# InternetMaximalism/plonky2_bn254

Measured on NVIDIA B200. Metric: g1_scalar_mul_stark_proofs_per_sec, higher is better.
Workload: dtype u64

## Files before the change

### plonky2_bn254_b200/csrc/merkle.cuh

```cuda
#pragma once
#include "poseidon.cuh"
#include "poseidon_tc.cuh"

namespace merkle {

using poseidon::Digest;

struct LeafHashK {
  const u64* lde;
  size_t stride;
  int W, log_n;
  Digest* out;
  int natural = 0;
  PB_HD void operator()(size_t j) const {
    u64 s[12];
#pragma unroll
    for (int i = 0; i < 12; i++) s[i] = 0;
    if (W <= 4) {
      for (int c = 0; c < W; c++) s[c] = lde[(size_t)c * stride + j];
    } else {
      int c = 0;
      for (; c + 8 <= W; c += 8) {
#pragma unroll
        for (int k = 0; k < 8; k++) s[k] = lde[(size_t)(c + k) * stride + j];
        poseidon::permute(s);
      }
      if (c < W) {
        for (int k = 0; c + k < W; k++) s[k] = lde[(size_t)(c + k) * stride + j];
        poseidon::permute(s);
      }
    }
    Digest d;
#pragma unroll
    for (int i = 0; i < 4; i++) d.e[i] = s[i];
    out[natural ? j : (size_t)gl::brev32((u32)j, log_n)] = d;
  }
};

struct RowHashK {
  const u64* rows;
  int len;
  Digest* out;
  PB_HD void operator()(size_t i) const {
    u64 s[12];
#pragma unroll
    for (int k = 0; k < 12; k++) s[k] = 0;
    const u64* row = rows + i * (size_t)len;
    if (len <= 4) {
      for (int c = 0; c < len; c++) s[c] = row[c];
    } else {
      for (int c = 0; c < len; c += 8) {
        for (int k = 0; k < 8 && c + k < len; k++) s[k] = row[c + k];
        poseidon::permute(s);
      }
    }
    Digest d;
#pragma unroll
    for (int k = 0; k < 4; k++) d.e[k] = s[k];
    out[i] = d;
  }
};

struct LevelK {
  const Digest* child;
  Digest* parent;
  PB_HD void operator()(size_t i) const { parent[i] = poseidon::two_to_one(child[2 * i], child[2 * i + 1]); }
};

#if !PB_HOSTSIM
__device__ __forceinline__ void stage_rc2(u64* rc2) {
  for (int i = threadIdx.x; i < poseidon::RC2_WORDS; i += blockDim.x) rc2[i] = poseidon::RC2_DEV[i];
  __syncthreads();
}

__global__ void __launch_bounds__(poseidon::tc::CTA, poseidon::tc::CTAS_PER_SM)
    k_leaf_hash_tc(const u64* __restrict__ lde, size_t stride, int W, int log_n, Digest* __restrict__ out, size_t rows,
                   int natural) {
  extern __shared__ unsigned char tc_dyn[];
  __shared__ u64 tc_bar;
  __shared__ u32 tc_slot[2];
  poseidon::tc::Ctx ctx;
  poseidon::tc::setup(ctx, tc_dyn, &tc_bar, tc_slot);
  const size_t j = (size_t)blockIdx.x * blockDim.x + threadIdx.x;
  const bool live = j < rows;
  const u64* p = lde + (live ? j : 0);
  u64 s[12];
#pragma unroll
  for (int i = 0; i < 12; i++) s[i] = 0;
  const int chunks = (W + 7) / 8;
#pragma unroll 1
  for (int c = 0; c < chunks; c++) {
    const int len = W - 8 * c;
    const u64* q = p + (size_t)c * 8 * stride;
#pragma unroll
    for (int k = 0; k < 8; k++)
      if (k < len) s[k] = q[(size_t)k * stride];
    poseidon::tc::permute(s, ctx);
  }
  if (live) {
    Digest d;
#pragma unroll
    for (int i = 0; i < 4; i++) d.e[i] = s[i];
    out[natural ? j : (size_t)gl::brev32((u32)j, log_n)] = d;
  }
  poseidon::tc::teardown(ctx);
}

__global__ void __launch_bounds__(128, 6) k_level(const Digest* __restrict__ child, Digest* __restrict__ parent, size_t n) {
  __shared__ __align__(16) u64 rc2[poseidon::RC2_WORDS];
  stage_rc2(rc2);
  const size_t i = (size_t)blockIdx.x * blockDim.x + threadIdx.x;
  if (i >= n) return;
  u64 s[12];
  const Digest l = child[2 * i], r = child[2 * i + 1];
#pragma unroll
  for (int k = 0; k < 4; k++) {
    s[k] = l.e[k];
    s[4 + k] = r.e[k];
    s[8 + k] = 0;
  }
  poseidon::lazy::permute(s, rc2);
  Digest d;
#pragma unroll
  for (int k = 0; k < 4; k++) d.e[k] = s[k];
  parent[i] = d;
}
#endif

static inline size_t tree_digests(int log_n, int cap_height) {
  size_t total = 0;
  for (int l = log_n; l >= cap_height; l--) total += (size_t)1 << l;
  return total;
}
static inline size_t level_offset(int log_n, int lvl) {
  size_t off = 0;
  for (int l = 0; l < lvl; l++) off += (size_t)1 << (log_n - l);
  return off;
}

static inline void launch_level(const Digest* child, Digest* parent, size_t n, pbStream s) {
#if PB_HOSTSIM
  LevelK k{child, parent};
  pb_launch("merkle level", k, n, s, 128);
#else
  k_level<<<(unsigned)((n + 127) / 128), 128, 0, s>>>(child, parent, n);
  g_pb_launches++;
  pb_check_last("merkle level");
#endif
}
static inline void build_levels(Digest* digests, int log_n, int cap_height, pbStream s) {
  if (cap_height > log_n) throw Pb254Error(6, "merkle: cap_height > log2(leaves)");
  size_t off = 0;
  for (int l = 0; l < log_n - cap_height; l++) {
    size_t m = (size_t)1 << (log_n - l);
    launch_level(digests + off, digests + off + m, m / 2, s);
    off += m;
  }
}

static inline void build_from_lde(const u64* lde, size_t stride, int W, int log_n, int cap_height, Digest* digests,
                                  pbStream s) {
#if PB_HOSTSIM
  LeafHashK k{lde, stride, W, log_n, digests};
  pb_launch("leaf hash", k, (size_t)1 << log_n, s, 128);
#else
  if (W <= 4) {
    LeafHashK k{lde, stride, W, log_n, digests};
    pb_launch("leaf copy", k, (size_t)1 << log_n, s, 128);
  } else {
    const size_t n = (size_t)1 << log_n;
    k_leaf_hash_tc<<<(unsigned)((n + 127) / 128), poseidon::tc::CTA, poseidon::tc::SMEM_BYTES, s>>>(lde, stride, W, log_n,
                                                                                                  digests, n, 0);
    g_pb_launches++;
    pb_check_last("leaf hash");
  }
#endif
  build_levels(digests, log_n, cap_height, s);
}
static inline void build_from_rows(const u64* rows, int len, int log_n, int cap_height, Digest* digests, pbStream s) {
  RowHashK k{rows, len, digests};
  pb_launch("row hash", k, (size_t)1 << log_n, s, 128);
  build_levels(digests, log_n, cap_height, s);
}


static inline void hash_rows_natural(const u64* m, size_t stride, int W, size_t rows, Digest* out, pbStream s) {
#if PB_HOSTSIM
  LeafHashK k{m, stride, W, 0, out, 1};
  pb_launch("leaf hash (rows)", k, rows, s, 128);
#else
  if (W <= 4) {
    LeafHashK k{m, stride, W, 0, out, 1};
    pb_launch("leaf copy (rows)", k, rows, s, 128);
  } else {
    k_leaf_hash_tc<<<(unsigned)((rows + 127) / 128), poseidon::tc::CTA, poseidon::tc::SMEM_BYTES, s>>>(m, stride, W, 0, out,
                                                                                                     rows, 1);
    g_pb_launches++;
    pb_check_last("leaf hash (rows)");
  }
#endif
}
struct SubtreeLeavesK {
  const Digest* all;
  Digest* leaves;
  size_t first;
  int log_N;
  PB_HD void operator()(size_t q) const { leaves[q] = all[gl::brev32((u32)(first + q), log_N)]; }
};

}
```

### plonky2_bn254_b200/csrc/poseidon_tc.cuh

```cuda
#pragma once
#include "poseidon.cuh"

#if !PB_HOSTSIM
namespace poseidon {
namespace tc {

static constexpr int CTA = 128;
static constexpr int A_BYTES = 128 * 128;
static constexpr int B_BYTES = 96 * 128;
static constexpr int CTAS_PER_SM = 5;
static constexpr int SMEM_BYTES = 41 * 1024;
static_assert(A_BYTES + 2 * B_BYTES + 1024 <= SMEM_BYTES && SMEM_BYTES <= 48 * 1024, "shared-memory plan");
__host__ __device__ constexpr u32 idesc(u32 n) { return (2u << 4) | ((n >> 3) << 17) | ((128u >> 4) << 24); }

static __device__ const uint4 B_IMAGE[B_BYTES / 16] = {
#include "poseidon_constants_tcb.inc"
};
static __device__ const uint4 BF_IMAGE[B_BYTES / 16] = {
#include "poseidon_constants_tcf.inc"
};

__device__ __forceinline__ u32 smem_u32(const void* p) { return (u32)__cvta_generic_to_shared(p); }

__device__ __forceinline__ u64 smem_desc(u32 addr) {
  return (u64)((addr & 0x3FFFFu) >> 4) | ((u64)(1024u >> 4) << 32) | (1ull << 46) | (2ull << 61);
}

struct Ctx {
  unsigned char* row;
  u32 r7;
  u32 bar;
  u32 tmem0, tmem1;
  u64 adesc, bdesc, bfdesc;
  u32 parity;
};

__device__ __forceinline__ void setup(Ctx& c, unsigned char* dyn, u64* bar, u32* slot) {
  const u32 t = threadIdx.x;
  unsigned char* base = dyn + ((1024u - (smem_u32(dyn) & 1023u)) & 1023u);
  unsigned char* a = base;
  unsigned char* b = base + A_BYTES;
  unsigned char* bf = b + B_BYTES;
  for (int i = t; i < B_BYTES / 16; i += CTA) {
    reinterpret_cast<uint4*>(b)[i] = B_IMAGE[i];
    reinterpret_cast<uint4*>(bf)[i] = BF_IMAGE[i];
  }
  c.row = a + t * 128;
  c.r7 = t & 7;
  c.bar = smem_u32(bar);
  if (t == 0) {
    asm volatile("mbarrier.init.shared::cta.b64 [%0], 1;" ::"r"(c.bar));
    asm volatile("fence.mbarrier_init.release.cluster;" ::: "memory");
  }
  if (t < 32) {
    asm volatile("tcgen05.alloc.cta_group::1.sync.aligned.shared::cta.b32 [%0], 64;" ::"r"(smem_u32(slot)) : "memory");
    asm volatile("tcgen05.alloc.cta_group::1.sync.aligned.shared::cta.b32 [%0], 32;" ::"r"(smem_u32(slot + 1)) : "memory");
    asm volatile("tcgen05.relinquish_alloc_permit.cta_group::1.sync.aligned;" ::: "memory");
  }
  asm volatile("tcgen05.fence::before_thread_sync;" ::: "memory");
  __syncthreads();
  asm volatile("tcgen05.fence::after_thread_sync;" ::: "memory");
  c.tmem0 = reinterpret_cast<volatile u32*>(slot)[0];
  c.tmem1 = reinterpret_cast<volatile u32*>(slot)[1];
  c.adesc = smem_desc(smem_u32(a));
  c.bdesc = smem_desc(smem_u32(b));
  c.bfdesc = smem_desc(smem_u32(bf));
  c.parity = 0;
}

__device__ __forceinline__ void teardown(const Ctx& c) {
  asm volatile("tcgen05.fence::before_thread_sync;" ::: "memory");
  __syncthreads();
  if (threadIdx.x < 32) {
    asm volatile("tcgen05.dealloc.cta_group::1.sync.aligned.b32 %0, 64;" ::"r"(c.tmem0) : "memory");
    asm volatile("tcgen05.dealloc.cta_group::1.sync.aligned.b32 %0, 32;" ::"r"(c.tmem1) : "memory");
  }
}

template <u32 N>
__device__ __forceinline__ void mma_i8(u32 d_tmem, u64 adesc, u64 bdesc, u32 accumulate) {
  asm volatile(
      "{\n\t"
      ".reg .pred p;\n\t"
      "setp.ne.b32 p, %4, 0;\n\t"
      "tcgen05.mma.cta_group::1.kind::i8 [%0], %1, %2, %3, p;\n\t"
      "}" ::"r"(d_tmem),
      "l"(adesc), "l"(bdesc), "n"(idesc(N)), "r"(accumulate)
      : "memory");
}

#define PB_TMEM_LD32(v, addr)                                                                                       \
  asm volatile(                                                                                                     \
      "tcgen05.ld.sync.aligned.32x32b.x32.b32 {%0, %1, %2, %3, %4, %5, %6, %7, %8, %9, %10, %11, %12, %13, %14, "   \
      "%15, %16, %17, %18, %19, %20, %21, %22, %23, %24, %25, %26, %27, %28, %29, %30, %31}, [%32];"                \
      : "=r"(v[0]), "=r"(v[1]), "=r"(v[2]), "=r"(v[3]), "=r"(v[4]), "=r"(v[5]), "=r"(v[6]), "=r"(v[7]), "=r"(v[8]), \
        "=r"(v[9]), "=r"(v[10]), "=r"(v[11]), "=r"(v[12]), "=r"(v[13]), "=r"(v[14]), "=r"(v[15]), "=r"(v[16]),      \
        "=r"(v[17]), "=r"(v[18]), "=r"(v[19]), "=r"(v[20]), "=r"(v[21]), "=r"(v[22]), "=r"(v[23]), "=r"(v[24]),     \
        "=r"(v[25]), "=r"(v[26]), "=r"(v[27]), "=r"(v[28]), "=r"(v[29]), "=r"(v[30]), "=r"(v[31])                   \
      : "r"(addr)                                                                                                   \
      : "memory")

__device__ __forceinline__ u64 recombine4(u32 acc0, u32 acc1, u32 acc2, u32 acc3) {
  const u32 t1 = __byte_perm(acc1, 0, 0x1044), u1 = __byte_perm(acc1, 0, 0x4432);
  const u32 t3 = __byte_perm(acc3, 0, 0x1044), u3 = __byte_perm(acc3, 0, 0x4432);
  u32 lo, hi;
  asm("{\n\t"
      ".reg .u32 w2, c;\n\t"
      "add.cc.u32   %0, %2, %3;\n\t"
      "addc.u32     %1, %4, %5;\n\t"
      "add.cc.u32   %1, %1, %6;\n\t"
      "addc.u32     w2, %7, 0;\n\t"
      "add.cc.u32   %1, %1, w2;\n\t"
      "addc.u32     c, 0, 0;\n\t"
      "sub.cc.u32   %0, %0, w2;\n\t"
      "subc.u32     %1, %1, 0;\n\t"
      "sub.u32      c, 0, c;\n\t"
      "add.cc.u32   %0, %0, c;\n\t"
      "addc.u32     %1, %1, 0;\n\t"
      "}"
      : "=&r"(lo), "=&r"(hi)
      : "r"(acc0), "r"(t1), "r"(u1), "r"(acc2), "r"(t3), "r"(u3));
  return ((u64)hi << 32) | lo;
}

__device__ __forceinline__ u64 fold8(const u32* q) {
  return recombine4(q[0] + (q[1] << 8), q[2] + (q[3] << 8), q[4] + (q[5] << 8), q[6] + (q[7] << 8));
}


__device__ __forceinline__ u32 onehot(int p, int w) { return (p >> 2) == w ? 1u << ((p & 3) * 8) : 0u; }

__device__ __forceinline__ u32 complement4(const u64 s[12], int i0, int i1, int i2, int i3) {
  const u32 a = __byte_perm((u32)(s[i0] >> 32), (u32)(s[i1] >> 32), 0x0073);
  const u32 b = __byte_perm((u32)(s[i2] >> 32), (u32)(s[i3] >> 32), 0x0073);
  return ~__byte_perm(a, b, 0x5410);
}

__device__ __forceinline__ void product(u64 s[12], Ctx& c, u64 bdesc, uint4 x6, uint4 x7) {
#pragma unroll
  for (int ch = 0; ch < 6; ch++)
    *reinterpret_cast<uint4*>(c.row + ((ch ^ c.r7) << 4)) =
        make_uint4((u32)s[2 * ch], (u32)(s[2 * ch] >> 32), (u32)s[2 * ch + 1], (u32)(s[2 * ch + 1] >> 32));
  *reinterpret_cast<uint4*>(c.row + ((6 ^ c.r7) << 4)) = x6;
  *reinterpret_cast<uint4*>(c.row + ((7 ^ c.r7) << 4)) = x7;
  asm volatile("fence.proxy.async.shared::cta;" ::: "memory");
  asm volatile("tcgen05.fence::before_thread_sync;" ::: "memory");
  __syncthreads();
  if (threadIdx.x == 0) {
    asm volatile("tcgen05.fence::after_thread_sync;" ::: "memory");
#pragma unroll
    for (int k = 0; k < 4; k++) {
      mma_i8<64>(c.tmem0, c.adesc + 2 * k, bdesc + 2 * k, k > 0);
      mma_i8<32>(c.tmem1, c.adesc + 2 * k, bdesc + (64 * 128 >> 4) + 2 * k, k > 0);
    }
    asm volatile("tcgen05.commit.cta_group::1.mbarrier::arrive::one.shared::cluster.b64 [%0];" ::"r"(c.bar) : "memory");
  }
  {
    u32 ok;
    do {
      asm volatile(
          "{\n\t"
          ".reg .pred p;\n\t"
          "mbarrier.try_wait.parity.shared::cta.b64 p, [%1], %2;\n\t"
          "selp.u32 %0, 1, 0, p;\n\t"
          "}"
          : "=r"(ok)
          : "r"(c.bar), "r"(c.parity)
          : "memory");
    } while (!ok);
    c.parity ^= 1;
  }
  asm volatile("tcgen05.fence::after_thread_sync;" ::: "memory");
  {
    const u32 lane_off = ((threadIdx.x >> 5) * 32u) << 16;
    const u32 t0 = c.tmem0 + lane_off, t1 = c.tmem0 + lane_off + 32, t2 = c.tmem1 + lane_off;
#define PB_TC_FOLD(a, base)                                                                                   \
  _Pragma("unroll") for (int r = 0; r < 4; r++) {                                                             \
    const u32* q = a + 8 * r;                                                                                 \
    s[base + r] = fold8(q);                                                                                   \
  }
    u32 a[32], b[32];
    PB_TMEM_LD32(a, t0);
    asm volatile("tcgen05.wait::ld.sync.aligned;" ::: "memory");
    PB_TMEM_LD32(b, t1);
    PB_TC_FOLD(a, 0)
    asm volatile("tcgen05.wait::ld.sync.aligned;" ::: "memory");
    PB_TMEM_LD32(a, t2);
    PB_TC_FOLD(b, 4)
    asm volatile("tcgen05.wait::ld.sync.aligned;" ::: "memory");
    PB_TC_FOLD(a, 8)
#undef PB_TC_FOLD
  }
}

__device__ __forceinline__ void permute(u64 s[12], Ctx& c) {
#pragma unroll
  for (int i = 0; i < 12; i++) {
    const u64 k = RC_DEV[i];
    u64 t = s[i] + k;
    if (t < k) t += gl::EPS;
    s[i] = t;
  }
  constexpr int N_FUSED = N_PARTIAL / 2, N_LAYERS = 2 * HALF_FULL + N_FUSED;
#pragma unroll 1
  for (int L = 0; L < N_LAYERS; L++) {
    uint4 x6, x7;
    u64 bdesc;
    if (L < HALF_FULL || L >= HALF_FULL + N_FUSED) {
#pragma unroll 1
      for (int j = 0; j < 2; j++) {
        u64 t[6];
#pragma unroll
        for (int i = 0; i < 6; i++) t[i] = lazy::sbox(s[i]);
#pragma unroll
        for (int i = 0; i < 6; i++) {
          s[i] = s[i + 6];
          s[i + 6] = t[i];
        }
      }
      const int R = L < HALF_FULL ? L : L + N_FUSED;
      const int p = R < N_ROUNDS - 1 ? R : -1;
      x6 = make_uint4(onehot(p, 0), onehot(p, 1), onehot(p, 2), onehot(p, 3));
      x7 = make_uint4(onehot(p, 4), onehot(p, 5), onehot(p, 6), onehot(p, 7));
      bdesc = c.bdesc;
    } else {
      const int j = L - HALF_FULL, r = HALF_FULL + 2 * j;
      s[0] = lazy::sbox(s[0]);
      u32 X[6][4];
#pragma unroll
      for (int k = 0; k < 6; k++) {
        const u32 a0 = (u32)s[2 * k], a1 = (u32)(s[2 * k] >> 32), b0 = (u32)s[2 * k + 1], b1 = (u32)(s[2 * k + 1] >> 32);
        X[k][0] = __byte_perm(a0, b0, 0x5410);
        X[k][1] = __byte_perm(a0, b0, 0x7632);
        X[k][2] = __byte_perm(a1, b1, 0x5410);
        X[k][3] = __byte_perm(a1, b1, 0x7632);
      }
      const uint4 k0 = *reinterpret_cast<const uint4*>(RC2_DEV + (r + 1) * 24);
      u32 acc[4] = {k0.x, k0.y, k0.z, k0.w};
      lazy::dp_row<0, 0>(acc, X);
      const u64 t = lazy::sbox(recombine4(acc[0], acc[1], acc[2], acc[3]));
      const int p = 8 + j;
      x6 = make_uint4((u32)t, (u32)(t >> 32), onehot(p, 2), onehot(p, 3));
      x7 = make_uint4(onehot(p, 4) | (~(u32)(s[0] >> 32) & 0xFF000000u), complement4(s, 1, 2, 3, 4),
                      complement4(s, 5, 6, 7, 8), complement4(s, 9, 10, 11, 11) & 0x00FFFFFFu);
      bdesc = c.bfdesc;
    }
    product(s, c, bdesc, x6, x7);
  }
#pragma unroll
  for (int i = 0; i < 12; i++) s[i] = s[i] >= gl::P ? s[i] - gl::P : s[i];
}

}
}
#endif
```

Measured before the change: 5.165.

## Interleave two leaf-hash sponges per thread to overlap tensor-core MMA with sbox work

The leaf-hash kernel now processes two rows per thread and ping-pongs their Poseidon permutations. While the tensor-core product for one state is in flight, the threads compute the sboxes for the other, hiding MMA latency and barrier stalls. The grid is halved and register pressure roughly doubles per thread, which may limit occupancy at the unchanged CTAs-per-SM bound.

```diff
diff --git a/plonky2_bn254_b200/csrc/merkle.cuh b/plonky2_bn254_b200/csrc/merkle.cuh
--- a/plonky2_bn254_b200/csrc/merkle.cuh
+++ b/plonky2_bn254_b200/csrc/merkle.cuh
@@ -3,6 +3,9 @@
 #include "poseidon_tc.cuh"
 
 namespace merkle {
+#ifndef LEAF_CTAS_PER_SM
+#define LEAF_CTAS_PER_SM 5
+#endif
 
 using poseidon::Digest;
 
@@ -73,7 +76,8 @@
   __syncthreads();
 }
 
-__global__ void __launch_bounds__(poseidon::tc::CTA, poseidon::tc::CTAS_PER_SM)
+static constexpr unsigned LEAF_ROWS_PER_CTA = 2 * poseidon::tc::CTA;
+__global__ void __launch_bounds__(poseidon::tc::CTA, LEAF_CTAS_PER_SM)
     k_leaf_hash_tc(const u64* __restrict__ lde, size_t stride, int W, int log_n, Digest* __restrict__ out, size_t rows,
                    int natural) {
   extern __shared__ unsigned char tc_dyn[];
@@ -81,27 +85,28 @@
   __shared__ u32 tc_slot[2];
   poseidon::tc::Ctx ctx;
   poseidon::tc::setup(ctx, tc_dyn, &tc_bar, tc_slot);
-  const size_t j = (size_t)blockIdx.x * blockDim.x + threadIdx.x;
-  const bool live = j < rows;
-  const u64* p = lde + (live ? j : 0);
-  u64 s[12];
-#pragma unroll
-  for (int i = 0; i < 12; i++) s[i] = 0;
-  const int chunks = (W + 7) / 8;
-#pragma unroll 1
-  for (int c = 0; c < chunks; c++) {
+  const size_t j0 = (size_t)blockIdx.x * LEAF_ROWS_PER_CTA + threadIdx.x, j1 = j0 + poseidon::tc::CTA;
+  const u64* p0 = lde + (j0 < rows ? j0 : 0);
+  const u64* p1 = lde + (j1 < rows ? j1 : 0);
+  u64 s[2][12];
+#pragma unroll
+  for (int i = 0; i < 12; i++) s[0][i] = s[1][i] = 0;
+  poseidon::tc::sponge2(s, ctx, (W + 7) / 8, [&](int g, int c, u64* sg) {
     const int len = W - 8 * c;
-    const u64* q = p + (size_t)c * 8 * stride;
+    const u64* q = (g ? p1 : p0) + (size_t)c * 8 * stride;
 #pragma unroll
     for (int k = 0; k < 8; k++)
-      if (k < len) s[k] = q[(size_t)k * stride];
-    poseidon::tc::permute(s, ctx);
-  }
-  if (live) {
-    Digest d;
-#pragma unroll
-    for (int i = 0; i < 4; i++) d.e[i] = s[i];
-    out[natural ? j : (size_t)gl::brev32((u32)j, log_n)] = d;
+      if (k < len) sg[k] = q[(size_t)k * stride];
+  });
+#pragma unroll
+  for (int g = 0; g < 2; g++) {
+    const size_t j = g ? j1 : j0;
+    if (j < rows) {
+      Digest d;
+#pragma unroll
+      for (int i = 0; i < 4; i++) d.e[i] = s[g][i];
+      out[natural ? j : (size_t)gl::brev32((u32)j, log_n)] = d;
+    }
   }
   poseidon::tc::teardown(ctx);
 }
@@ -169,7 +174,7 @@
     pb_launch("leaf copy", k, (size_t)1 << log_n, s, 128);
   } else {
     const size_t n = (size_t)1 << log_n;
-    k_leaf_hash_tc<<<(unsigned)((n + 127) / 128), poseidon::tc::CTA, poseidon::tc::SMEM_BYTES, s>>>(lde, stride, W, log_n,
+    k_leaf_hash_tc<<<(unsigned)((n + LEAF_ROWS_PER_CTA - 1) / LEAF_ROWS_PER_CTA), poseidon::tc::CTA, poseidon::tc::SMEM_BYTES, s>>>(lde, stride, W, log_n,
                                                                                                   digests, n, 0);
     g_pb_launches++;
     pb_check_last("leaf hash");
@@ -193,7 +198,7 @@
     LeafHashK k{m, stride, W, 0, out, 1};
     pb_launch("leaf copy (rows)", k, rows, s, 128);
   } else {
-    k_leaf_hash_tc<<<(unsigned)((rows + 127) / 128), poseidon::tc::CTA, poseidon::tc::SMEM_BYTES, s>>>(m, stride, W, 0, out,
+    k_leaf_hash_tc<<<(unsigned)((rows + LEAF_ROWS_PER_CTA - 1) / LEAF_ROWS_PER_CTA), poseidon::tc::CTA, poseidon::tc::SMEM_BYTES, s>>>(m, stride, W, 0, out,
                                                                                                      rows, 1);
     g_pb_launches++;
     pb_check_last("leaf hash (rows)");
diff --git a/plonky2_bn254_b200/csrc/poseidon_tc.cuh b/plonky2_bn254_b200/csrc/poseidon_tc.cuh
--- a/plonky2_bn254_b200/csrc/poseidon_tc.cuh
+++ b/plonky2_bn254_b200/csrc/poseidon_tc.cuh
@@ -136,7 +136,7 @@
   return ~__byte_perm(a, b, 0x5410);
 }
 
-__device__ __forceinline__ void product(u64 s[12], Ctx& c, u64 bdesc, uint4 x6, uint4 x7) {
+__device__ __forceinline__ void store_row(const Ctx& c, const u64 s[12], uint4 x6, uint4 x7) {
 #pragma unroll
   for (int ch = 0; ch < 6; ch++)
     *reinterpret_cast<uint4*>(c.row + ((ch ^ c.r7) << 4)) =
@@ -144,17 +144,19 @@
   *reinterpret_cast<uint4*>(c.row + ((6 ^ c.r7) << 4)) = x6;
   *reinterpret_cast<uint4*>(c.row + ((7 ^ c.r7) << 4)) = x7;
   asm volatile("fence.proxy.async.shared::cta;" ::: "memory");
-  asm volatile("tcgen05.fence::before_thread_sync;" ::: "memory");
-  __syncthreads();
-  if (threadIdx.x == 0) {
-    asm volatile("tcgen05.fence::after_thread_sync;" ::: "memory");
-#pragma unroll
-    for (int k = 0; k < 4; k++) {
-      mma_i8<64>(c.tmem0, c.adesc + 2 * k, bdesc + 2 * k, k > 0);
-      mma_i8<32>(c.tmem1, c.adesc + 2 * k, bdesc + (64 * 128 >> 4) + 2 * k, k > 0);
-    }
-    asm volatile("tcgen05.commit.cta_group::1.mbarrier::arrive::one.shared::cluster.b64 [%0];" ::"r"(c.bar) : "memory");
-  }
+}
+
+__device__ __forceinline__ void issue(const Ctx& c, u64 bdesc) {
+  asm volatile("tcgen05.fence::after_thread_sync;" ::: "memory");
+#pragma unroll
+  for (int k = 0; k < 4; k++) {
+    mma_i8<64>(c.tmem0, c.adesc + 2 * k, bdesc + 2 * k, k > 0);
+    mma_i8<32>(c.tmem1, c.adesc + 2 * k, bdesc + (64 * 128 >> 4) + 2 * k, k > 0);
+  }
+  asm volatile("tcgen05.commit.cta_group::1.mbarrier::arrive::one.shared::cluster.b64 [%0];" ::"r"(c.bar) : "memory");
+}
+
+__device__ __forceinline__ void wait_fold(u64 s[12], Ctx& c) {
   {
     u32 ok;
     do {
@@ -193,7 +195,18 @@
   }
 }
 
-__device__ __forceinline__ void permute(u64 s[12], Ctx& c) {
+__device__ __forceinline__ void product(u64 s[12], Ctx& c, u64 bdesc, uint4 x6, uint4 x7) {
+  store_row(c, s, x6, x7);
+  asm volatile("tcgen05.fence::before_thread_sync;" ::: "memory");
+  __syncthreads();
+  if (threadIdx.x == 0) issue(c, bdesc);
+  wait_fold(s, c);
+}
+
+static constexpr int N_FUSED = N_PARTIAL / 2, N_LAYERS = 2 * HALF_FULL + N_FUSED;
+__host__ __device__ constexpr bool fused_layer(int L) { return L >= HALF_FULL && L < HALF_FULL + N_FUSED; }
+
+__device__ __forceinline__ void add_rc0(u64 s[12]) {
 #pragma unroll
   for (int i = 0; i < 12; i++) {
     const u64 k = RC_DEV[i];
@@ -201,54 +214,127 @@
     if (t < k) t += gl::EPS;
     s[i] = t;
   }
-  constexpr int N_FUSED = N_PARTIAL / 2, N_LAYERS = 2 * HALF_FULL + N_FUSED;
+}
+
+__device__ __forceinline__ void canonicalize(u64 s[12]) {
+#pragma unroll
+  for (int i = 0; i < 12; i++) s[i] = s[i] >= gl::P ? s[i] - gl::P : s[i];
+}
+
+__device__ __forceinline__ u64 layer_sboxes(u64 s[12], int L) {
+  if (!fused_layer(L)) {
+#pragma unroll 1
+    for (int j = 0; j < 2; j++) {
+      u64 t[6];
+#pragma unroll
+      for (int i = 0; i < 6; i++) t[i] = lazy::sbox(s[i]);
+#pragma unroll
+      for (int i = 0; i < 6; i++) {
+        s[i] = s[i + 6];
+        s[i + 6] = t[i];
+      }
+    }
+    return 0;
+  } else {
+    const int j = L - HALF_FULL, r = HALF_FULL + 2 * j;
+    s[0] = lazy::sbox(s[0]);
+    u32 X[6][4];
+#pragma unroll
+    for (int k = 0; k < 6; k++) {
+      const u32 a0 = (u32)s[2 * k], a1 = (u32)(s[2 * k] >> 32), b0 = (u32)s[2 * k + 1], b1 = (u32)(s[2 * k + 1] >> 32);
+      X[k][0] = __byte_perm(a0, b0, 0x5410);
+      X[k][1] = __byte_perm(a0, b0, 0x7632);
+      X[k][2] = __byte_perm(a1, b1, 0x5410);
+      X[k][3] = __byte_perm(a1, b1, 0x7632);
+    }
+    const uint4 k0 = *reinterpret_cast<const uint4*>(RC2_DEV + (r + 1) * 24);
+    u32 acc[4] = {k0.x, k0.y, k0.z, k0.w};
+    lazy::dp_row<0, 0>(acc, X);
+    return lazy::sbox(recombine4(acc[0], acc[1], acc[2], acc[3]));
+  }
+}
+
+__device__ __forceinline__ void layer_tail(const u64 s[12], int L, u64 t, uint4& x6, uint4& x7) {
+  if (!fused_layer(L)) {
+    const int R = L < HALF_FULL ? L : L + N_FUSED;
+    const int p = R < N_ROUNDS - 1 ? R : -1;
+    x6 = make_uint4(onehot(p, 0), onehot(p, 1), onehot(p, 2), onehot(p, 3));
+    x7 = make_uint4(onehot(p, 4), onehot(p, 5), onehot(p, 6), onehot(p, 7));
+  } else {
+    const int p = 8 + L - HALF_FULL;
+    x6 = make_uint4((u32)t, (u32)(t >> 32), onehot(p, 2), onehot(p, 3));
+    x7 = make_uint4(onehot(p, 4) | (~(u32)(s[0] >> 32) & 0xFF000000u), complement4(s, 1, 2, 3, 4),
+                    complement4(s, 5, 6, 7, 8), complement4(s, 9, 10, 11, 11) & 0x00FFFFFFu);
+  }
+}
+
+__device__ __forceinline__ void store_layer(const Ctx& c, const u64 s[12], int L, u64 t) {
+  uint4 x6, x7;
+  layer_tail(s, L, t, x6, x7);
+  store_row(c, s, x6, x7);
+}
+
+__device__ __forceinline__ void permute(u64 s[12], Ctx& c) {
+  add_rc0(s);
 #pragma unroll 1
   for (int L = 0; L < N_LAYERS; L++) {
     uint4 x6, x7;
-    u64 bdesc;
-    if (L < HALF_FULL || L >= HALF_FULL + N_FUSED) {
+    layer_tail(s, L, layer_sboxes(s, L), x6, x7);
+    product(s, c, fused_layer(L) ? c.bfdesc : c.bdesc, x6, x7);
+  }
+  canonicalize(s);
+}
+
+template <class Absorb>
+__device__ __forceinline__ void sponge2(u64 (&s)[2][12], Ctx& c, int chunks, Absorb&& absorb) {
+  u64 t[2];
+#pragma unroll
+  for (int g = 0; g < 2; g++) {
+    absorb(g, 0, s[g]);
+    add_rc0(s[g]);
+    t[g] = layer_sboxes(s[g], 0);
+  }
+  store_layer(c, s[0], 0, t[0]);
+  asm volatile("tcgen05.fence::before_thread_sync;" ::: "memory");
+  __syncthreads();
+  if (threadIdx.x == 0) issue(c, c.bdesc);
+  const int steps = 2 * chunks * N_LAYERS;
+  int L = 0, k = 0;
 #pragma unroll 1
-      for (int j = 0; j < 2; j++) {
-        u64 t[6];
-#pragma unroll
-        for (int i = 0; i < 6; i++) t[i] = lazy::sbox(s[i]);
-#pragma unroll
-        for (int i = 0; i < 6; i++) {
-          s[i] = s[i + 6];
-          s[i + 6] = t[i];
-        }
+  for (int i = 0; i < steps; i++) {
+    const int g = i & 1;
+    const int nL = L + 1 == N_LAYERS ? 0 : L + 1;
+    const bool more = i + 2 < steps;
+    wait_fold(s[0], c);
+    const bool next = i + 1 < steps;
+    if (next) store_layer(c, s[1], g == 0 ? L : nL, t[1]);
+    asm volatile("tcgen05.fence::before_thread_sync;" ::: "memory");
+    __syncthreads();
+    if (threadIdx.x == 0 && next) issue(c, fused_layer(g == 0 ? L : nL) ? c.bfdesc : c.bdesc);
+    if (more) {
+      if (nL == 0) {
+        canonicalize(s[0]);
+        absorb(g, k + 1, s[0]);
+        add_rc0(s[0]);
       }
-      const int R = L < HALF_FULL ? L : L + N_FUSED;
-      const int p = R < N_ROUNDS - 1 ? R : -1;
-      x6 = make_uint4(onehot(p, 0), onehot(p, 1), onehot(p, 2), onehot(p, 3));
-      x7 = make_uint4(onehot(p, 4), onehot(p, 5), onehot(p, 6), onehot(p, 7));
-      bdesc = c.bdesc;
-    } else {
-      const int j = L - HALF_FULL, r = HALF_FULL + 2 * j;
-      s[0] = lazy::sbox(s[0]);
-      u32 X[6][4];
-#pragma unroll
-      for (int k = 0; k < 6; k++) {
-        const u32 a0 = (u32)s[2 * k], a1 = (u32)(s[2 * k] >> 32), b0 = (u32)s[2 * k + 1], b1 = (u32)(s[2 * k + 1] >> 32);
-        X[k][0] = __byte_perm(a0, b0, 0x5410);
-        X[k][1] = __byte_perm(a0, b0, 0x7632);
-        X[k][2] = __byte_perm(a1, b1, 0x5410);
-        X[k][3] = __byte_perm(a1, b1, 0x7632);
-      }
-      const uint4 k0 = *reinterpret_cast<const uint4*>(RC2_DEV + (r + 1) * 24);
-      u32 acc[4] = {k0.x, k0.y, k0.z, k0.w};
-      lazy::dp_row<0, 0>(acc, X);
-      const u64 t = lazy::sbox(recombine4(acc[0], acc[1], acc[2], acc[3]));
-      const int p = 8 + j;
-      x6 = make_uint4((u32)t, (u32)(t >> 32), onehot(p, 2), onehot(p, 3));
-      x7 = make_uint4(onehot(p, 4) | (~(u32)(s[0] >> 32) & 0xFF000000u), complement4(s, 1, 2, 3, 4),
-                      complement4(s, 5, 6, 7, 8), complement4(s, 9, 10, 11, 11) & 0x00FFFFFFu);
-      bdesc = c.bfdesc;
-    }
-    product(s, c, bdesc, x6, x7);
-  }
-#pragma unroll
-  for (int i = 0; i < 12; i++) s[i] = s[i] >= gl::P ? s[i] - gl::P : s[i];
+      t[0] = layer_sboxes(s[0], nL);
+    }
+    if (g == 1) {
+      if (nL == 0) k++;
+      L = nL;
+    }
+#pragma unroll
+    for (int j = 0; j < 12; j++) {
+      const u64 x = s[0][j];
+      s[0][j] = s[1][j];
+      s[1][j] = x;
+    }
+    const u64 x = t[0];
+    t[0] = t[1];
+    t[1] = x;
+  }
+  canonicalize(s[0]);
+  canonicalize(s[1]);
 }
 
 }
```

Measured after the change: 5.050 (median of 6 runs). 2.2% lower.
